# drwangxian/viterbi_spl

Measured on AMD Instinct MI355X. Metric: Viterbi Mframes/s at S=361 T=30k; achieved HBM GB/s vs peak, higher is better.
Workload: dtype f32

## Files before the change

### viterbi_spl_amd/csrc/banded.hip

```cpp
#include "device_common.hpp"

namespace vit {

template <int W, int NWT, bool DW, bool DBG, int NXT, typename ET>
__global__ void __launch_bounds__((NWT + (DW ? 3 : 2)) * 64) banded_forward_kernel(FwdArgs a) {
    extern __shared__ __align__(16) unsigned char smem[];
    constexpr int NP = NWT * 64;
    constexpr int EPL = NWT;
    const int S = a.S, SP = a.SP, T = a.T, SD = a.SD;
    constexpr int DC = NP + 16;
    float* dls = reinterpret_cast<float*>(smem);
    float* dl = dls + 4;
    float* Pv = dls + 4 * DC;
    float* Sv = Pv + NP + 1;
    float* Dv = Sv + NP + 1;
    VI* tot = reinterpret_cast<VI*>(Dv + kMaxDenseRows);

    const int tid = threadIdx.x;
    const int lane = tid & 63;
    const int wv = __builtin_amdgcn_readfirstlane(tid >> 6);
    const int song = blockIdx.x;
    const int Tb = song_length(a.lengths, song, T);
    const ET* __restrict__ E = reinterpret_cast<const ET*>(a.logE) + (size_t)song * T * S;
    float* __restrict__ hist = a.hist + (size_t)song * T * SD;
    constexpr bool GEN = NXT < 0;
    constexpr int NXL = GEN ? kMaxExtras : NXT;
    const int nx = GEN ? a.n_extras : NXT, nd = GEN ? a.n_dense : 0;
#ifdef VIT_TIMING_HOOKS
    const int dbg = DBG ? a.debug : 0;
#else
    constexpr int dbg = 0;
#endif

    const bool is_target = wv < NWT;
    const int j = tid;
    const bool tvalid = is_target && j < S;
    const int jst = j < S ? j : S + 1;
    const int jld = j < S ? j : S - 1;
    const int jc = j < SP ? j : 0;
    int lo = 0, kind = -2;
    float cj = 0.f;
    float aw[W];
    float xa[kMaxExtras];
    int xcol[kMaxExtras];
#pragma unroll
    for (int k = 0; k < kMaxExtras; ++k) { xa[k] = -INFINITY; xcol[k] = a.extras[k]; }
#pragma unroll
    for (int w = 0; w < W; ++w) aw[w] = 0.f;
    if (is_target) {
        cj = reinterpret_cast<const float*>(a.image + a.off_rowc)[jc];
        lo = reinterpret_cast<const int32_t*>(a.image + a.off_lo)[jc];
        kind = j < SP ? reinterpret_cast<const int32_t*>(a.image + a.off_kind)[jc] : -2;
        const float* __restrict__ tab = reinterpret_cast<const float*>(a.image + a.off_tabA);
        const float* __restrict__ xaT = reinterpret_cast<const float*>(a.image + a.off_extraA);
#pragma unroll
        for (int w = 0; w < W; ++w) aw[w] = tab[(size_t)w * SP + jc];
#pragma unroll
        for (int k = 0; k < kMaxExtras; ++k) xa[k] = xaT[(size_t)k * SP + jc];
    }
    const int role = wv - NWT;
    constexpr int kDenseRole = DW ? 2 : 1;
    const int blk = role == 1 ? 63 - lane : lane;
    const int i0 = blk * EPL;
    bool smask[EPL];
    float dA[kMaxDenseRows][EPL];
    {
        const float* __restrict__ daT = reinterpret_cast<const float*>(a.image + a.off_denseA);
#pragma unroll
        for (int e = 0; e < EPL; ++e) {
            const int i = i0 + e;
            bool m = i >= S;
#pragma unroll
            for (int k = 0; k < kMaxExtras; ++k) m |= (k < nx && i == xcol[k]);
            smask[e] = m;
#pragma unroll
            for (int d = 0; d < kMaxDenseRows; ++d)
                dA[d][e] = (role == kDenseRole && i < S && d < nd) ? daT[(size_t)d * SP + i] : -INFINITY;
        }
    }

    for (int k = tid; k < 4 * DC; k += blockDim.x) dls[k] = -INFINITY;
    __syncthreads();
    if (is_target) {
        if (tvalid) {
            const float d = reinterpret_cast<const float*>(a.image + a.off_logpi)[j] + load_e<ET>(E + j);
            hist[j] = d;
#pragma unroll
            for (int c = 0; c < 4; ++c) dl[c * DC + j - c] = d;
        }
    } else if (lane == 0) {
        if (role == 0) Pv[0] = -INFINITY;
        if (role == 1) Sv[NP] = -INFINITY;
    }
    float e_a = (tvalid && Tb > 1) ? load_e<ET>(E + S + j) : 0.f;
    float e_b = (tvalid && Tb > 2) ? load_e<ET>(E + 2 * (size_t)S + j) : 0.f;
#pragma unroll
    for (int w = 0; w < W; ++w) asm volatile("" ::"v"(aw[w]));
#pragma unroll
    for (int k = 0; k < kMaxExtras; ++k) asm volatile("" ::"v"(xa[k]));
#pragma unroll
    for (int e = 0; e < EPL; ++e) {
#pragma unroll
        for (int d = 0; d < kMaxDenseRows; ++d) asm volatile("" ::"v"(dA[d][e]));
    }
    asm volatile("" ::"v"(lo), "v"(kind), "v"(cj), "v"(e_a), "v"(e_b));
    __syncthreads();

    unsigned long long ph0 = 0, ph1 = 0, ph2 = 0, ph3 = 0;
    auto stamp = [&]() -> unsigned long long {
        unsigned long long v;
        asm volatile("s_memtime %0\n\ts_waitcnt lgkmcnt(0)" : "=s"(v)::"memory");
        return v;
    };
    auto frame = [&](const int t, float& e_slot) {
        float m = -INFINITY;
        const bool prof = (dbg & 256) != 0;
        const unsigned long long s0 = prof ? stamp() : 0ull;
        if (is_target) {
            float m0 = -INFINITY, m1 = -INFINITY, m2 = -INFINITY, m3 = -INFINITY;
            float xd[NXL > 0 ? NXL : 1];
#pragma unroll
            for (int k = 0; k < NXL; ++k) xd[k] = (!GEN || k < nx) ? dl[xcol[k]] : -INFINITY;
            if (!(dbg & 1)) {
                const f32x4* __restrict__ win = reinterpret_cast<const f32x4*>(dl + (lo & 3) * DC + (lo & ~3));
#pragma unroll
                for (int w = 0; w + 7 < W; w += 8) {
                    const f32x4 da = win[w / 4], db = win[w / 4 + 1];
                    const f32x2 c0_ = f32x2{da.x, da.y} + f32x2{aw[w + 0], aw[w + 1]};
                    const f32x2 c1_ = f32x2{da.z, da.w} + f32x2{aw[w + 2], aw[w + 3]};
                    const f32x2 c2_ = f32x2{db.x, db.y} + f32x2{aw[w + 4], aw[w + 5]};
                    const f32x2 c3_ = f32x2{db.z, db.w} + f32x2{aw[w + 6], aw[w + 7]};
                    m0 = fmaxf(fmaxf(m0, c0_.x), c0_.y);
                    m1 = fmaxf(fmaxf(m1, c1_.x), c1_.y);
                    m2 = fmaxf(fmaxf(m2, c2_.x), c2_.y);
                    m3 = fmaxf(fmaxf(m3, c3_.x), c3_.y);
                }
            }
#pragma unroll
            for (int k = 0; k < NXL; ++k) m1 = fmaxf(m1, xd[k] + xa[k]);
            m = fmaxf(fmaxf(m0, m1), fmaxf(m2, m3));
        } else if (!(dbg & 2)) {
            float d[EPL];
#pragma unroll
            for (int e = 0; e < EPL; ++e) d[e] = dl[i0 + e];
            if (role == 0) {
                float p[EPL];
                float run = -INFINITY;
#pragma unroll
                for (int e = 0; e < EPL; ++e) {
                    run = fmaxf(run, smask[e] ? -INFINITY : d[e]);
                    p[e] = run;
                }
                const float inc = wave_scan_max(run);
                const float ex = wave_shift_up(inc, -INFINITY);
#pragma unroll
                for (int e = 0; e < EPL; ++e) Pv[i0 + e + 1] = fmaxf(ex, p[e]);
                if (lane == 63 && !(dbg & 8)) hist[(size_t)(t - 1) * SD + S] = inc;
            } else {
                if (role == 1) {
                    float p[EPL];
                    float run = -INFINITY;
#pragma unroll
                    for (int e = EPL - 1; e >= 0; --e) {
                        run = fmaxf(run, smask[e] ? -INFINITY : d[e]);
                        p[e] = run;
                    }
                    const float ex = wave_shift_up(wave_scan_max(run), -INFINITY);
#pragma unroll
                    for (int e = 0; e < EPL; ++e) Sv[i0 + e] = fmaxf(ex, p[e]);
                }
                if (GEN && role == kDenseRole) {
#pragma unroll
                    for (int dr = 0; dr < kMaxDenseRows; ++dr) {
                        if (dr < nd) {
                            float dm = -INFINITY;
#pragma unroll
                            for (int e = 0; e < EPL; ++e) dm = fmaxf(dm, d[e] + dA[dr][e]);
                            dm = wave_max_all(dm);
                            if (lane == 0) Dv[dr] = dm;
                        }
                    }
                }
            }
        }
        const unsigned long long s1 = prof ? stamp() : 0ull;
        __syncthreads();
        const unsigned long long s2 = prof ? stamp() : 0ull;

        if (is_target && !(dbg & 4)) {
            m = fmaxf(m, fmaxf(Pv[lo], Sv[lo + W]) + cj);
            if (GEN) {
                const float dres = Dv[kind >= 0 ? kind : 0];
                if (kind >= 0) m = dres;
            }
            {
                const float dn = tvalid ? m + e_slot : -INFINITY;
#pragma unroll
                for (int c = 0; c < 4; ++c) dl[c * DC + j - c] = dn;
                if (!(dbg & 8)) {
                    float* __restrict__ hrow = hist + (size_t)t * SD;
                    const int tn = t + 2 < Tb ? t + 2 : Tb - 1;
                    const ET* __restrict__ erow = E + (size_t)tn * S;
                    hrow[jst] = dn;
                    e_slot = load_e<ET>(erow + jld);
                }
            }
        }
        const unsigned long long s3 = prof ? stamp() : 0ull;
        __syncthreads();
        if (prof) {
            const unsigned long long s4 = stamp();
            ph0 += s1 - s0; ph1 += s2 - s1; ph2 += s3 - s2; ph3 += s4 - s3;
        }
    };
    const unsigned long long clk0 = (dbg & 48) ? __builtin_amdgcn_s_memtime() : 0ull;
    const unsigned long long rt0 = (dbg & 48) ? __builtin_amdgcn_s_memrealtime() : 0ull;
    int t = 1;
    for (; t + 1 < Tb; t += 2) {
        frame(t, e_a);
        frame(t + 1, e_b);
    }
    if (t < Tb) frame(t, e_a);

    terminal_argmax(is_target ? dl[j] : -INFINITY, j, tvalid, tot, NWT + (DW ? 3 : 2), a.last_state, a.loglik, song);
    if ((dbg & 256) && lane == 0 && Tb > 1) {
        float* o = a.fmax + (size_t)song * 64 + 4 * wv;
        const float n = (float)(Tb - 1);
        o[0] = (float)ph0 / n; o[1] = (float)ph1 / n; o[2] = (float)ph2 / n; o[3] = (float)ph3 / n;
    }
    if ((dbg & 48) && tid == 0) {
        const unsigned long long d = (dbg & 16) ? __builtin_amdgcn_s_memtime() - clk0 : __builtin_amdgcn_s_memrealtime() - rt0;
        a.fmax[(size_t)song * 64 + 63] = (float)d / (float)(Tb > 1 ? Tb - 1 : 1);
    }
}

#include "banded_floor.inc"

template <int NXT, int PF, typename ET, bool WPR = false>
__global__ void __launch_bounds__(64 * (kSplitFullWaves + kSplitHalfWaves)) banded_floor_split_forward_kernel(FwdArgs a) {
    extern __shared__ __align__(16) unsigned char smem[];
    constexpr int W = 32;
    constexpr int NWF = kSplitFullWaves, NW = kSplitFullWaves + kSplitHalfWaves;
    using L = FloorSplitLds;
    constexpr int DC = L::DC, BUF = L::BUF;
    float* dls = reinterpret_cast<float*>(smem) + L::dls;
    float* fmg = dls + L::fmg;
    VI* tot = reinterpret_cast<VI*>(dls + L::tot);
    const int S = a.S, SP = a.SP, T = a.T, SD = a.SD;
    constexpr bool GEN = NXT < 0;
    constexpr int NXL = GEN ? kMaxExtras : NXT;
    const int nx = GEN ? a.n_extras : NXT;

    const int tid = threadIdx.x;
    const int lane = tid & 63;
    const int wv = __builtin_amdgcn_readfirstlane(tid >> 6);
    const bool half = wv >= NWF;
    const int hh = half ? lane >> 5 : 0;
    const int song = blockIdx.x;
    const int Tb = song_length(a.lengths, song, T);
    const ET* __restrict__ E = reinterpret_cast<const ET*>(a.logE) + (size_t)song * T * S;
    float* __restrict__ hist = a.hist + (size_t)song * T * SD;

    const int j = half ? 64 * NWF + 32 * (wv - NWF) + (lane & 31) : tid;
    const bool tvalid = j < S;
    const bool own = tvalid && hh == 0;
    const int jc = tvalid ? j : 0;
    const int jld = tvalid ? j : S - 1;
    const bool is_fm = j == S;
    const unsigned hoff = tvalid ? (unsigned)(SD + j) : (is_fm ? (unsigned)S : (unsigned)(SD + S + 1));
    const unsigned hoffb = 4u * hoff, eoffb = (unsigned)(sizeof(ET) * jld);
    const int lo = reinterpret_cast<const int32_t*>(a.image + a.off_lo)[jc];
    int xcol[NXL > 0 ? NXL : 1];
    bool is_x = false;
#pragma unroll
    for (int k = 0; k < NXL; ++k) {
        xcol[k] = k < nx ? a.extras[k] : 0;
        is_x |= (k < nx && j == xcol[k]);
    }
    const int sh = a.win_shift;
    const int lov = (tvalid ? lo : 0) + sh;
    const float* rp = dls + 4 + (lov & 3) * DC + (lov & ~3) + 16 * hh;
    float* fmp = fmg + fm_slot(lane);

    for (int k = tid; k < L::reset; k += NW * 64) dls[k] = -INFINITY;
    __syncthreads();

#ifdef VIT_TIMING_HOOKS
    const bool probe = (a.debug & 48) != 0;
    constexpr bool wprobe = WPR;
    WaveProbe wp_;
#else
    constexpr bool probe = false;
#endif
    unsigned long long clk0 = 0ull, rt0 = 0ull;

    auto body = [&](auto role, auto resets) {
        constexpr bool HALF = decltype(role)::value, RESETS = decltype(resets)::value;
        constexpr int WL = HALF ? W / 2 : W;
        const float cj = own ? reinterpret_cast<const float*>(a.image + a.off_rowc)[jc] : -INFINITY;
        float aw[WL];
        float xa[NXL > 0 ? NXL : 1];
        {
            const float* __restrict__ tab = reinterpret_cast<const float*>(a.image + a.off_tabA);
            const float* __restrict__ xaT = reinterpret_cast<const float*>(a.image + a.off_extraA);
#pragma unroll
            for (int w = 0; w < WL; ++w) aw[w] = tvalid ? tab[(size_t)(w + (HALF ? 16 * hh : 0)) * SP + jc] : -INFINITY;
#pragma unroll
            for (int k = 0; k < NXL; ++k)
                xa[k] = (tvalid && k < nx && (!HALF || hh == 1)) ? xaT[(size_t)k * SP + jc] : -INFINITY;
        }
        float* wp = dls + 4 + sh + j + (HALF ? hh * split_upper_off(DC) : 0);
        int xo[NXL > 0 ? NXL : 1];
#pragma unroll
        for (int k = 0; k < NXL; ++k) {
            xo[k] = 4 + sh + xcol[k];
            asm volatile("" : "+v"(xo[k]));
        }

        auto produce = [&](const float dn, const int WB, const int G, const int Z) {
#pragma unroll
            for (int c = 0; c < (HALF ? 2 : 4); ++c) wp[WB * BUF + floor_copy_off(DC, c)] = dn;
            fm_publish(fmp + G * kFmGroupFloats, (NXL > 0 && is_x) ? -INFINITY : dn);
            if constexpr (RESETS) fmg[Z * kFmGroupFloats + lane] = -INFINITY;
        };

        {
            const float d0 = tvalid ? reinterpret_cast<const float*>(a.image + a.off_logpi)[j] + load_e<ET>(E + j) : -INFINITY;
            if (own) hist[j] = d0;
            produce(d0, 0, 0, 1);
        }
        float er[PF];
#pragma unroll
        for (int k = 0; k < PF; ++k) er[k] = load_e<ET>(E + (size_t)(1 + k < Tb ? 1 + k : Tb - 1) * S + jld);
#pragma unroll
        for (int w = 0; w < WL; ++w) asm volatile("" ::"v"(aw[w]));
#pragma unroll
        for (int k = 0; k < NXL; ++k) asm volatile("" ::"v"(xa[k]));
        asm volatile("" ::"v"(cj));
        __syncthreads();

        const unsigned rowH = 4u * (unsigned)SD, rowE = (unsigned)sizeof(ET) * (unsigned)S;
        float* hb = hist;
        const ET* eb = E;
        unsigned elim = 0;
        auto round_bases = [&](const int t) {
            const int r = t + PF < Tb ? t + PF : Tb - 1;
            const int ahead = Tb - 1 - r < PF ? Tb - 1 - r : PF;
            hb = hist + (size_t)(t - 1) * SD;
            eb = E + (size_t)r * S;
            elim = (unsigned)ahead * rowE;
        };
        auto frame = [&](float& e_slot, const int u) {
            const int RB = u & 1, WB = RB ^ 1;
            const int GR = u % kFmGroups, GW = (u + 1) % kFmGroups, GZ = (u + 2) % kFmGroups;
            const f32x4* __restrict__ win = reinterpret_cast<const f32x4*>(rp + RB * BUF);
            float xd[NXL > 0 ? NXL : 1];
            f32x4 fq;
            float m0, m1 = -INFINITY, m2 = -INFINITY, m3 = -INFINITY;
#pragma unroll
            for (int k = 0; k < NXL; ++k) xd[k] = dls[xo[k] + RB * BUF];
            fq = reinterpret_cast<const f32x4*>(fmg + GR * kFmGroupFloats)[0];
            asm volatile("" ::: "memory");
            f32x4 dw[WL / 4];
#pragma unroll
            for (int q = 0; q < WL / 4; ++q) dw[q] = win[q];
            __builtin_amdgcn_sched_barrier(0);
            const float M = fmaxf(fmaxf(fq.x, fq.y), fmaxf(fq.z, fq.w));
            m0 = M + cj;
            __builtin_amdgcn_sched_barrier(0);
#pragma unroll
            for (int w = 0; w < WL; w += 8) {
                const f32x4 da = dw[w / 4], db = dw[w / 4 + 1];
                f32x2 c0_ = f32x2{da.x, da.y} + f32x2{aw[w + 0], aw[w + 1]};
                f32x2 c1_ = f32x2{da.z, da.w} + f32x2{aw[w + 2], aw[w + 3]};
                f32x2 c2_ = f32x2{db.x, db.y} + f32x2{aw[w + 4], aw[w + 5]};
                f32x2 c3_ = f32x2{db.z, db.w} + f32x2{aw[w + 6], aw[w + 7]};
                asm volatile("" : "+v"(c0_), "+v"(c1_), "+v"(c2_), "+v"(c3_));
                m0 = fmaxf(fmaxf(m0, c0_.x), c0_.y);
                m1 = fmaxf(fmaxf(m1, c1_.x), c1_.y);
                m2 = fmaxf(fmaxf(m2, c2_.x), c2_.y);
                m3 = fmaxf(fmaxf(m3, c3_.x), c3_.y);
            }
#pragma unroll
            for (int k = 0; k < NXL; ++k) m1 = fmaxf(m1, xd[k] + xa[k]);
            float mx = fmaxf(fmaxf(m0, m1), fmaxf(m2, m3));
            if constexpr (HALF) mx = max_other_half(mx);
            const float dn = mx + e_slot;
#ifdef VIT_TIMING_HOOKS
            if constexpr (wprobe) wp_.before_publish(dn);
#endif
            produce(dn, WB, GW, GZ);
            asm volatile("" ::: "memory");
            const unsigned eso = (unsigned)u * rowE < elim ? (unsigned)u * rowE : elim;
            row_store_f32(hb, hoffb, (HALF && is_fm) ? M : dn, (unsigned)u * rowH);
            e_slot = row_load_e<ET>(eb, eoffb, eso);
#ifdef VIT_TIMING_HOOKS
            if constexpr (wprobe) wp_.barrier(); else
#endif
            __syncthreads();
        };
#ifdef VIT_TIMING_HOOKS
        if constexpr (wprobe) wp_.start();
#endif
        clk0 = probe ? __builtin_amdgcn_s_memtime() : 0ull;
        rt0 = probe ? __builtin_amdgcn_s_memrealtime() : 0ull;
        int t = 1;
        for (; t + PF - 1 < Tb; t += PF) {
            round_bases(t);
#pragma unroll
            for (int k = 0; k < PF; ++k) frame(er[k], k);
        }
        round_bases(t);
#pragma unroll
        for (int k = 0; k < PF - 1; ++k)
            if (t + k < Tb) frame(er[k], k);
    };
    static_assert(PF % 2 == 0 && PF % kFmGroups == 0, "the unrolled frames must cycle through whole buffer and slot-group rounds");
    if (!half) body(std::false_type{}, std::false_type{});
    else if (wv == NW - 1) body(std::true_type{}, std::true_type{});
    else body(std::true_type{}, std::false_type{});

    const int fb = (Tb - 1) & 1;
    terminal_argmax(own ? dls[4 + sh + fb * BUF + j] : -INFINITY, j, own, tot, NW, a.last_state, a.loglik, song);
    if (probe && tid == 0) {
        const unsigned long long d = (a.debug & 16) ? __builtin_amdgcn_s_memtime() - clk0 : __builtin_amdgcn_s_memrealtime() - rt0;
        a.fmax[(size_t)song * 64 + 63] = (float)d / (float)(Tb > 1 ? Tb - 1 : 1);
    }
#ifdef VIT_TIMING_HOOKS
    if constexpr (wprobe) wp_.finish(a.fmax + (size_t)song * 64, wv, lane, Tb - 1);
#endif
}

template <int NPW>
struct FloorPairLds {
    static constexpr int NP = NPW * 128;
    static constexpr int DC = NP + 16;
    static constexpr int BUF = 4 * DC;
    static constexpr int NWM = (NPW + 3) / 4 * 4;
    static constexpr int dls = 0;
    static constexpr int wm = dls + 2 * BUF;
    static constexpr int reset = wm + 2 * NWM;
    static constexpr int dump = reset;
    static constexpr int tot = dump + 64 + NWM;
    static constexpr int end = tot + 16 * (int)(sizeof(VI) / sizeof(float));
    static_assert(sizeof(float) * end <= kLdsBytes, "one workgroup's LDS");
    static constexpr size_t bytes() { return sizeof(float) * end; }
};

template <int W, int NPW, int NXT, int PF, typename ET>
__global__ void __launch_bounds__(NPW * 64) banded_floor_pair_forward_kernel(FwdArgs a) {
    extern __shared__ __align__(16) unsigned char smem[];
    using L = FloorPairLds<NPW>;
    constexpr int DC = L::DC, BUF = L::BUF, NWM = L::NWM;
    float* dls = reinterpret_cast<float*>(smem) + L::dls;
    float* wm = dls + L::wm;
    float* dump = dls + L::dump;
    VI* tot = reinterpret_cast<VI*>(dls + L::tot);
    const int S = a.S, SP = a.SP, T = a.T, SD = a.SD;
    constexpr bool GEN = NXT < 0;
    constexpr int NXL = GEN ? kMaxExtras : NXT;
    const int nx = GEN ? a.n_extras : NXT;

    const int tid = threadIdx.x;
    const int lane = tid & 63;
    const int wv = __builtin_amdgcn_readfirstlane(tid >> 6);
    const int song = blockIdx.x;
    const int Tb = song_length(a.lengths, song, T);
    const ET* __restrict__ E = reinterpret_cast<const ET*>(a.logE) + (size_t)song * T * S;
    float* __restrict__ hist = a.hist + (size_t)song * T * SD;

    const int j0 = 2 * tid, j1 = 2 * tid + 1;
    const bool v0 = j0 < S, v1 = j1 < S;
    const int jc0 = v0 ? j0 : 0, jc1 = v1 ? j1 : jc0;
    const int jl0 = v0 ? j0 : S - 1, jl1 = v1 ? j1 : S - 1;
    const unsigned hoff0 = v0 ? (unsigned)(SD + j0) : (j0 == S ? (unsigned)S : (unsigned)(SD + S + 1));
    const unsigned hoff1 = v1 ? (unsigned)(SD + j1) : (j1 == S ? (unsigned)S : (unsigned)(SD + S + 1));
    const bool fm0 = j0 == S, fm1 = j1 == S;
    const int lo2 = v0 ? reinterpret_cast<const int32_t*>(a.image + a.off_lo2)[jc0 >> 1] : 0;
    const float* __restrict__ rc = reinterpret_cast<const float*>(a.image + a.off_rowc);
    f32x2 cj = f32x2{v0 ? rc[jc0] : -INFINITY, v1 ? rc[jc1] : -INFINITY};
    float aw0[W], aw1[W];
    f32x2 xa[NXL > 0 ? NXL : 1];
    int xcol[NXL > 0 ? NXL : 1];
    bool x0 = false, x1 = false;
    {
        const float* __restrict__ tab = reinterpret_cast<const float*>(a.image + a.off_tabP);
        const float* __restrict__ xaT = reinterpret_cast<const float*>(a.image + a.off_extraA);
#pragma unroll
        for (int w = 0; w < W; ++w) {
            aw0[w] = v0 ? tab[(size_t)w * SP + jc0] : -INFINITY;
            aw1[w] = v1 ? tab[(size_t)w * SP + jc1] : -INFINITY;
        }
#pragma unroll
        for (int k = 0; k < NXL; ++k) {
            xcol[k] = k < nx ? a.extras[k] : 0;
            xa[k] = f32x2{(v0 && k < nx) ? xaT[(size_t)k * SP + jc0] : -INFINITY, (v1 && k < nx) ? xaT[(size_t)k * SP + jc1] : -INFINITY};
            x0 |= (k < nx && j0 == xcol[k]);
            x1 |= (k < nx && j1 == xcol[k]);
        }
    }
    const int sh = a.win_shift2;
    const int lov = lo2 + sh;
    const float* rp = dls + 4 + (lov & 3) * DC + (lov & ~3);
    float* wp = dls + 4 + sh + j0;
    float* wmp = lane == 63 ? wm + wv : dump + lane;

    for (int k = tid; k < L::reset; k += NPW * 64) dls[k] = -INFINITY;
    __syncthreads();

    auto produce = [&](const f32x2 dn, const int WB) {
#pragma unroll
        for (int c = 0; c < 4; ++c) {
            wp[WB * BUF + c * DC - c] = dn.x;
            wp[WB * BUF + c * DC - c + 1] = dn.y;
        }
        const float inc = wave_scan_max(fmaxf((NXL > 0 && x0) ? -INFINITY : dn.x, (NXL > 0 && x1) ? -INFINITY : dn.y));
        wmp[WB * NWM] = inc;
    };

    {
        const float* __restrict__ lpi = reinterpret_cast<const float*>(a.image + a.off_logpi);
        f32x2 d0 = f32x2{-INFINITY, -INFINITY};
        if (v0) { d0.x = lpi[j0] + load_e<ET>(E + j0); hist[j0] = d0.x; }
        if (v1) { d0.y = lpi[j1] + load_e<ET>(E + j1); hist[j1] = d0.y; }
        produce(d0, 0);
    }
    f32x2 er[PF];
#pragma unroll
    for (int k = 0; k < PF; ++k) {
        const ET* __restrict__ row = E + (size_t)(1 + k < Tb ? 1 + k : Tb - 1) * S;
        er[k] = f32x2{load_e<ET>(row + jl0), load_e<ET>(row + jl1)};
    }
#pragma unroll
    for (int w = 0; w < W; ++w) asm volatile("" ::"v"(aw0[w]), "v"(aw1[w]));
#pragma unroll
    for (int k = 0; k < NXL; ++k) asm volatile("" ::"v"(xa[k]));
    asm volatile("" ::"v"(cj));
    __syncthreads();

    auto frame = [&](const int t, f32x2& e_slot, const int RB) {
        const int WB = RB ^ 1;
        const f32x4* __restrict__ win = reinterpret_cast<const f32x4*>(rp + RB * BUF);
        float xd[NXL > 0 ? NXL : 1];
#pragma unroll
        for (int k = 0; k < NXL; ++k) xd[k] = dls[4 + sh + RB * BUF + xcol[k]];
        f32x4 wq[NWM / 4];
#pragma unroll
        for (int q = 0; q < NWM / 4; ++q) wq[q] = reinterpret_cast<const f32x4*>(wm + RB * NWM)[q];
        f32x4 dw[W / 4];
#pragma unroll
        for (int q = 0; q < W / 4; ++q) dw[q] = win[q];
        float m0 = -INFINITY, m1 = -INFINITY, n0 = -INFINITY, n1 = -INFINITY;
#pragma unroll
        for (int w = 0; w + 3 < W; w += 4) {
            const f32x4 d = dw[w / 4];
            const f32x2 a0 = f32x2{d.x, d.y} + f32x2{aw0[w + 0], aw0[w + 1]};
            const f32x2 a1 = f32x2{d.z, d.w} + f32x2{aw0[w + 2], aw0[w + 3]};
            const f32x2 b0 = f32x2{d.x, d.y} + f32x2{aw1[w + 0], aw1[w + 1]};
            const f32x2 b1 = f32x2{d.z, d.w} + f32x2{aw1[w + 2], aw1[w + 3]};
            m0 = fmaxf(fmaxf(m0, a0.x), a0.y);
            n0 = fmaxf(fmaxf(n0, a1.x), a1.y);
            m1 = fmaxf(fmaxf(m1, b0.x), b0.y);
            n1 = fmaxf(fmaxf(n1, b1.x), b1.y);
        }
        float M = fmaxf(fmaxf(wq[0].x, wq[0].y), fmaxf(wq[0].z, wq[0].w));
#pragma unroll
        for (int q = 1; q < NWM / 4; ++q) M = fmaxf(fmaxf(fmaxf(M, wq[q].x), wq[q].y), fmaxf(wq[q].z, wq[q].w));
        const f32x2 fl = f32x2{M, M} + cj;
        m0 = fmaxf(m0, fl.x);
        m1 = fmaxf(m1, fl.y);
#pragma unroll
        for (int k = 0; k < NXL; ++k) {
            const f32x2 xv = f32x2{xd[k], xd[k]} + xa[k];
            n0 = fmaxf(n0, xv.x);
            n1 = fmaxf(n1, xv.y);
        }
        const f32x2 dn = f32x2{fmaxf(m0, n0), fmaxf(m1, n1)} + e_slot;
        produce(dn, WB);
        asm volatile("" ::: "memory");
        const int tn = t + PF < Tb ? t + PF : Tb - 1;
        float* __restrict__ hb = hist + (size_t)(t - 1) * SD;
        const ET* __restrict__ erow = E + (size_t)tn * S;
        hb[hoff0] = fm0 ? M : dn.x;
        hb[hoff1] = fm1 ? M : dn.y;
        e_slot = f32x2{load_e<ET>(erow + jl0), load_e<ET>(erow + jl1)};
        __syncthreads();
    };
#ifdef VIT_TIMING_HOOKS
    const bool probe = (a.debug & 48) != 0;
#else
    constexpr bool probe = false;
#endif
    const unsigned long long clk0 = probe ? __builtin_amdgcn_s_memtime() : 0ull;
    const unsigned long long rt0 = probe ? __builtin_amdgcn_s_memrealtime() : 0ull;
    int t = 1;
    for (; t + PF - 1 < Tb; t += PF) {
#pragma unroll
        for (int k = 0; k < PF; ++k) frame(t + k, er[k], k & 1);
    }
#pragma unroll
    for (int k = 0; k < PF - 1; ++k)
        if (t + k < Tb) frame(t + k, er[k], k & 1);

    {
        const int fb = (Tb - 1) & 1;
        const float* fin = dls + 4 + sh + fb * BUF;
        VI x = vi_identity();
        if (v0) x = VI{fin[j0], j0};
        if (v1) x = op_fwd(x, VI{fin[j1], j1});
        x = wave_scan<false>(x);
        if (lane == 63) tot[wv] = x;
        __syncthreads();
        if (tid == 0) {
            VI acc = vi_identity();
            for (int b = 0; b < NPW; ++b) acc = op_fwd(acc, tot[b]);
            if (acc.i == kBig) acc.i = 0;
            a.last_state[song] = acc.i;
            if (a.loglik) a.loglik[song] = acc.v;
        }
    }
    if (probe && tid == 0) {
        const unsigned long long d = (a.debug & 16) ? __builtin_amdgcn_s_memtime() - clk0 : __builtin_amdgcn_s_memrealtime() - rt0;
        a.fmax[(size_t)song * 64 + 63] = (float)d / (float)(Tb > 1 ? Tb - 1 : 1);
    }
}

__global__ void scan_selftest_kernel(const float* __restrict__ vals, int mode, float* __restrict__ out_v,
                                     int32_t* __restrict__ out_i) {
    const int j = threadIdx.x + blockIdx.x * blockDim.x;
    VI x{vals[j], (int)threadIdx.x};
    if (mode == 0) x = wave_scan<false>(x);
    else if (mode == 1) x = wave_scan<true>(x);
    else if (mode == 2) x.v = wave_scan_max(x.v);
    else if (mode == 3) x.v = wave_shift_up(wave_scan_max(x.v), -INFINITY);
    else x.v = wave_max_all(x.v);
    out_v[j] = x.v;
    out_i[j] = x.i;
}

template <int W, int NWT, typename ET>
static hipError_t launch_floor_t(const FwdArgs& a, hipStream_t st) {
    constexpr int PF = floor_pf<W>();
    if constexpr (W == 32 && NWT == 6) {
        static_assert(kSplitStates == NWT * 64, "the split kernel keeps the six-wave kernel's LDS and history layout");
        if (a.fwd_form == 6 || (a.fwd_form == 0 && a.B <= 256 && std::is_same_v<ET, float>)) {
            constexpr size_t ldss = FloorSplitLds::bytes();
            constexpr int NWS = kSplitFullWaves + kSplitHalfWaves;
#ifdef VIT_TIMING_HOOKS
            if ((a.debug & 64) && a.n_extras == 1)
                hipLaunchKernelGGL((banded_floor_split_forward_kernel<1, PF, ET, true>), dim3((int)a.B), dim3(NWS * 64), ldss, st, a);
            else
#endif
            if (a.n_extras == 1)
                hipLaunchKernelGGL((banded_floor_split_forward_kernel<1, PF, ET>), dim3((int)a.B), dim3(NWS * 64), ldss, st, a);
            else
                hipLaunchKernelGGL((banded_floor_split_forward_kernel<-1, PF, ET>), dim3((int)a.B), dim3(NWS * 64), ldss, st, a);
            return hipGetLastError();
        }
    }
    if constexpr (W <= 32 && NWT <= 8) {
        const bool pair = a.pair_ok && ((a.B > 256 && a.fwd_form != 1 && a.fwd_form != 6) || a.fwd_form == 2);
        if (pair) {
            constexpr int NPW = (NWT + 1) / 2;
            constexpr int PFP = 4;
            constexpr size_t ldsp = FloorPairLds<NPW>::bytes();
            if (W == 32 && a.n_extras == 1)
                hipLaunchKernelGGL((banded_floor_pair_forward_kernel<W, NPW, (W == 32 ? 1 : -1), PFP, ET>), dim3((int)a.B), dim3(NPW * 64), ldsp, st, a);
            else
                hipLaunchKernelGGL((banded_floor_pair_forward_kernel<W, NPW, -1, PFP, ET>), dim3((int)a.B), dim3(NPW * 64), ldsp, st, a);
            return hipGetLastError();
        }
    }
    constexpr size_t ldsf = FloorLds<W, NWT>::bytes();
#ifdef VIT_TIMING_HOOKS
    if constexpr (W == 32 && NWT == 6) {
        if ((a.debug & 64) && a.n_extras == 1) {
            hipLaunchKernelGGL((banded_floor_forward_kernel<W, NWT, 1, PF, ET, WgVariant::Plain, true>), dim3((int)a.B), dim3(NWT * 64), ldsf, st, a);
            return hipGetLastError();
        }
    }
#endif
    return with_nxt<W>(a.n_extras, [&](auto nxt) {
        hipLaunchKernelGGL((banded_floor_forward_kernel<W, NWT, decltype(nxt)::value, PF, ET>), dim3((int)a.B), dim3(NWT * 64), ldsf, st, a);
        return hipGetLastError();
    });
}

template <int W, int NWT, typename ET>
static hipError_t launch_scan_t(const FwdArgs& a, hipStream_t st) {
    constexpr int NP = NWT * 64;
    const size_t lds = sizeof(float) * (4 * (NP + 16) + 2 * (NP + 1) + kMaxDenseRows) + sizeof(VI) * 16;
    if (a.n_dense > 0 && a.B <= 256)
        hipLaunchKernelGGL((banded_forward_kernel<W, NWT, true, false, -1, ET>), dim3((int)a.B), dim3((NWT + 3) * 64), lds, st, a);
#ifdef VIT_TIMING_HOOKS
    else if (a.debug)
        hipLaunchKernelGGL((banded_forward_kernel<W, NWT, false, true, -1, ET>), dim3((int)a.B), dim3((NWT + 2) * 64), lds, st, a);
#endif
    else if (W == 32 && a.n_dense == 0 && a.n_extras == 1)
        hipLaunchKernelGGL((banded_forward_kernel<W, NWT, false, false, (W == 32 ? 1 : -1), ET>), dim3((int)a.B), dim3((NWT + 2) * 64), lds, st, a);
    else if (W == 32 && a.n_dense == 0 && a.n_extras == 0)
        hipLaunchKernelGGL((banded_forward_kernel<W, NWT, false, false, (W == 32 ? 0 : -1), ET>), dim3((int)a.B), dim3((NWT + 2) * 64), lds, st, a);
    else
        hipLaunchKernelGGL((banded_forward_kernel<W, NWT, false, false, -1, ET>), dim3((int)a.B), dim3((NWT + 2) * 64), lds, st, a);
    return hipGetLastError();
}

template <int W, int NWT, typename ET>
static hipError_t launch_banded_t(const FwdArgs& a, hipStream_t st) {
    const bool floor_ok = a.floor_ok && a.S < NWT * 64 && a.fwd_form != 3 && !(a.debug & ~112);
    if constexpr (floor_form_instantiated(W, NWT)) {
        if (floor_ok) return launch_floor_t<W, NWT, ET>(a, st);
    }
    if constexpr (scan_form_instantiated(W, NWT)) return launch_scan_t<W, NWT, ET>(a, st);
    return hipErrorInvalidConfiguration;
}

hipError_t launch_banded(const FwdArgs& a, bool f16, hipStream_t st) {
    auto go = [&](auto et) {
        using ET = decltype(et);
        return dispatch_width(a.W, [&](auto w) {
            return dispatch_waves(a.S, [&](auto n) { return launch_banded_t<decltype(w)::value, decltype(n)::value, ET>(a, st); });
        });
    };
    return f16 ? go(__half{}) : go(float{});
}

static hipError_t floor_variant(const FwdArgs& a, WgVariant v, bool f16, hipStream_t st, int* per_cu) {
    switch (v) {
        case WgVariant::Packed: return f16 ? floor_variant_e<__half, WgVariant::Packed>(a, st, per_cu) : floor_variant_e<float, WgVariant::Packed>(a, st, per_cu);
        case WgVariant::Ckpt: return f16 ? floor_variant_e<__half, WgVariant::Ckpt>(a, st, per_cu) : floor_variant_e<float, WgVariant::Ckpt>(a, st, per_cu);
        case WgVariant::PackedCkpt: return floor_pckpt(a, f16, st, per_cu);
        default: return hipErrorInvalidValue;
    }
}

hipError_t launch_banded_variant(const FwdArgs& a, WgVariant v, bool f16, hipStream_t st) {
    if (!wg_variant_args_ok(a, v, 2)) return hipErrorInvalidValue;
    return floor_variant(a, v, f16, st, nullptr);
}

hipError_t banded_variant_resident(const FwdArgs& a, WgVariant v, bool f16, int* per_cu) { return floor_variant(a, v, f16, nullptr, per_cu); }

hipError_t launch_scan_selftest(const float* vals, int n_waves, int mode, float* out_v, int32_t* out_i,
                                hipStream_t st) {
    hipLaunchKernelGGL(scan_selftest_kernel, dim3(n_waves), dim3(64), 0, st, vals, mode, out_v, out_i);
    return hipGetLastError();
}

}
```

Before: 459.9.

## Add explicit split waitcnts, half-wave priority, and idle-quad extra-column slot in split kernel

The frame loop becomes compile-time unrolled through integer sequences, so each frame and window group knows its index as a constant. That lets the code issue precise s_waitcnt values for vm and lgkm counters on the last window groups instead of relying on compiler-inserted waits. Half waves raise their scheduling priority. When the single extra column is the last state and lands in an idle quad, it publishes its value to a redirected max slot rather than masking it to -inf. The precise waits risk correctness if the counter bounds are wrong, and the extra-column path depends on a launcher-side condition.

```diff
diff --git a/viterbi_spl_amd/csrc/banded.hip b/viterbi_spl_amd/csrc/banded.hip
--- a/viterbi_spl_amd/csrc/banded.hip
+++ b/viterbi_spl_amd/csrc/banded.hip
@@ -236,7 +236,11 @@
 
 #include "banded_floor.inc"
 
-template <int NXT, int PF, typename ET, bool WPR = false>
+constexpr int split_waitcnt(int vm, int lgkm) { return (vm & 15) | ((vm >> 4) << 14) | (7 << 4) | (lgkm << 8); }
+constexpr int kNoVmWait = 63;
+template <int... K, typename F>
+__device__ __forceinline__ void split_frames(std::integer_sequence<int, K...>, F&& f) { (f(std::integral_constant<int, K>{}), ...); }
+template <int NXT, int PF, typename ET, bool WPR = false, bool XQ = false>
 __global__ void __launch_bounds__(64 * (kSplitFullWaves + kSplitHalfWaves)) banded_floor_split_forward_kernel(FwdArgs a) {
     extern __shared__ __align__(16) unsigned char smem[];
     constexpr int W = 32;
@@ -280,7 +284,8 @@
     const int sh = a.win_shift;
     const int lov = (tvalid ? lo : 0) + sh;
     const float* rp = dls + 4 + (lov & 3) * DC + (lov & ~3) + 16 * hh;
-    float* fmp = fmg + fm_slot(lane);
+    float* fmp = fmg + fm_slot((XQ && is_x) ? (lane | 1) : lane);
+    static_assert(!XQ || NXT == 1, "the extra column leaves M by address only where the launcher proved its quad idle");
 
     for (int k = tid; k < L::reset; k += NW * 64) dls[k] = -INFINITY;
     __syncthreads();
@@ -320,7 +325,7 @@
         auto produce = [&](const float dn, const int WB, const int G, const int Z) {
 #pragma unroll
             for (int c = 0; c < (HALF ? 2 : 4); ++c) wp[WB * BUF + floor_copy_off(DC, c)] = dn;
-            fm_publish(fmp + G * kFmGroupFloats, (NXL > 0 && is_x) ? -INFINITY : dn);
+            fm_publish(fmp + G * kFmGroupFloats, (!XQ && NXL > 0 && is_x) ? -INFINITY : dn);
             if constexpr (RESETS) fmg[Z * kFmGroupFloats + lane] = -INFINITY;
         };
 
@@ -350,7 +355,8 @@
             eb = E + (size_t)r * S;
             elim = (unsigned)ahead * rowE;
         };
-        auto frame = [&](float& e_slot, const int u) {
+        auto frame = [&](float& e_slot, auto uc) {
+            constexpr int u = decltype(uc)::value;
             const int RB = u & 1, WB = RB ^ 1;
             const int GR = u % kFmGroups, GW = (u + 1) % kFmGroups, GZ = (u + 2) % kFmGroups;
             const f32x4* __restrict__ win = reinterpret_cast<const f32x4*>(rp + RB * BUF);
@@ -367,10 +373,19 @@
             __builtin_amdgcn_sched_barrier(0);
             const float M = fmaxf(fmaxf(fq.x, fq.y), fmaxf(fq.z, fq.w));
             m0 = M + cj;
+            asm volatile("" ::"v"(m0));
             __builtin_amdgcn_sched_barrier(0);
-#pragma unroll
-            for (int w = 0; w < WL; w += 8) {
-                const f32x4 da = dw[w / 4], db = dw[w / 4 + 1];
+            split_frames(std::make_integer_sequence<int, WL / 8>{}, [&](auto gc) {
+                constexpr int w = 8 * decltype(gc)::value;
+                constexpr bool last = w + 8 == WL;
+                constexpr int vmw = PF - 1 + u;
+                static_assert(vmw <= 2 * (PF - 1) && 2 * (PF - 1) < kNoVmWait, "vmcnt bound: one store and one load per frame, 6-bit field");
+                constexpr bool pairw = w + 16 >= WL && w >= 8;
+                f32x4 da = dw[w / 4], db = dw[w / 4 + 1];
+                if constexpr (pairw) {
+                    __builtin_amdgcn_s_waitcnt(split_waitcnt(last ? vmw : kNoVmWait, last ? 0 : 2));
+                    asm volatile("" : "+v"(da), "+v"(db));
+                }
                 f32x2 c0_ = f32x2{da.x, da.y} + f32x2{aw[w + 0], aw[w + 1]};
                 f32x2 c1_ = f32x2{da.z, da.w} + f32x2{aw[w + 2], aw[w + 3]};
                 f32x2 c2_ = f32x2{db.x, db.y} + f32x2{aw[w + 4], aw[w + 5]};
@@ -380,7 +395,7 @@
                 m1 = fmaxf(fmaxf(m1, c1_.x), c1_.y);
                 m2 = fmaxf(fmaxf(m2, c2_.x), c2_.y);
                 m3 = fmaxf(fmaxf(m3, c3_.x), c3_.y);
-            }
+            });
 #pragma unroll
             for (int k = 0; k < NXL; ++k) m1 = fmaxf(m1, xd[k] + xa[k]);
             float mx = fmaxf(fmaxf(m0, m1), fmaxf(m2, m3));
@@ -389,10 +404,11 @@
 #ifdef VIT_TIMING_HOOKS
             if constexpr (wprobe) wp_.before_publish(dn);
 #endif
+            const float sv = (HALF && is_fm) ? M : dn;
+            const unsigned eso = (unsigned)u * rowE < elim ? (unsigned)u * rowE : elim;
             produce(dn, WB, GW, GZ);
             asm volatile("" ::: "memory");
-            const unsigned eso = (unsigned)u * rowE < elim ? (unsigned)u * rowE : elim;
-            row_store_f32(hb, hoffb, (HALF && is_fm) ? M : dn, (unsigned)u * rowH);
+            row_store_f32(hb, hoffb, sv, (unsigned)u * rowH);
             e_slot = row_load_e<ET>(eb, eoffb, eso);
 #ifdef VIT_TIMING_HOOKS
             if constexpr (wprobe) wp_.barrier(); else
@@ -404,16 +420,16 @@
 #endif
         clk0 = probe ? __builtin_amdgcn_s_memtime() : 0ull;
         rt0 = probe ? __builtin_amdgcn_s_memrealtime() : 0ull;
+        if constexpr (HALF) __builtin_amdgcn_s_setprio(1);
         int t = 1;
         for (; t + PF - 1 < Tb; t += PF) {
             round_bases(t);
-#pragma unroll
-            for (int k = 0; k < PF; ++k) frame(er[k], k);
+            split_frames(std::make_integer_sequence<int, PF>{}, [&](auto k) { frame(er[k], k); });
         }
         round_bases(t);
-#pragma unroll
-        for (int k = 0; k < PF - 1; ++k)
+        split_frames(std::make_integer_sequence<int, PF - 1>{}, [&](auto k) {
             if (t + k < Tb) frame(er[k], k);
+        });
     };
     static_assert(PF % 2 == 0 && PF % kFmGroups == 0, "the unrolled frames must cycle through whole buffer and slot-group rounds");
     if (!half) body(std::false_type{}, std::false_type{});
@@ -646,12 +662,17 @@
         if (a.fwd_form == 6 || (a.fwd_form == 0 && a.B <= 256 && std::is_same_v<ET, float>)) {
             constexpr size_t ldss = FloorSplitLds::bytes();
             constexpr int NWS = kSplitFullWaves + kSplitHalfWaves;
-#ifdef VIT_TIMING_HOOKS
-            if ((a.debug & 64) && a.n_extras == 1)
+            const bool xq = a.n_extras == 1 && a.extras[0] == a.S - 1 && (a.S - 1) % 4 == 0;
+#ifdef VIT_TIMING_HOOKS
+            if ((a.debug & 64) && xq)
+                hipLaunchKernelGGL((banded_floor_split_forward_kernel<1, PF, ET, true, true>), dim3((int)a.B), dim3(NWS * 64), ldss, st, a);
+            else if ((a.debug & 64) && a.n_extras == 1)
                 hipLaunchKernelGGL((banded_floor_split_forward_kernel<1, PF, ET, true>), dim3((int)a.B), dim3(NWS * 64), ldss, st, a);
             else
 #endif
-            if (a.n_extras == 1)
+            if (xq)
+                hipLaunchKernelGGL((banded_floor_split_forward_kernel<1, PF, ET, false, true>), dim3((int)a.B), dim3(NWS * 64), ldss, st, a);
+            else if (a.n_extras == 1)
                 hipLaunchKernelGGL((banded_floor_split_forward_kernel<1, PF, ET>), dim3((int)a.B), dim3(NWS * 64), ldss, st, a);
             else
                 hipLaunchKernelGGL((banded_floor_split_forward_kernel<-1, PF, ET>), dim3((int)a.B), dim3(NWS * 64), ldss, st, a);
```

Measured after the change: 488.2 (median of 6 runs). +6.1%, better.
